# VIS4ROB-lab/ccm_slam

Hardware: AMD Instinct MI355X
Metric: global-BA LM iterations/s (4-agent merged map) (higher is better)
Workload: dtype f64; 1 GPU; gba_c4: global BA (MapFusionGBA numerics), 2000 KFs / 150000 landmarks / 954782 observations, Huber sqrt(5.99), landmark-sharded x1

## Files before the change

ccm_slam_amd/csrc/ba.hip:

```cpp
#include "common.h"
#include "test_internal.h"
#include "ba_types.h"
#include "lane_xor.h"
#include "ba_math.h"
#include <algorithm>
#include <chrono>
#include <cmath>
#include <cstring>
#include <limits>
#include <numeric>

int ccm_allreduce_f64(ccm_ctx* ctx, double* d_buf, size_t n);
int ccm_allreduce_max_f64(ccm_ctx* ctx, double* d_buf, size_t n);

namespace {


inline double now_ms() {
  return std::chrono::duration<double, std::milli>(std::chrono::steady_clock::now().time_since_epoch()).count();
}

__device__ __forceinline__ double wave_sum(double v) { return lanex::wave_sum(v); }

__device__ __forceinline__ double block_sum(double v, double* lds ) {
// ... 218 lines not shown
      for (int k = 0; k < 12; k++) Jj[k] = 0.0;
    }
    if (d.E4) {
      v2d* E = reinterpret_cast<v2d*>(d.E4 + 4 * (size_t)s);
      v2d ea, eb; ea[0] = Xc[0]; ea[1] = Xc[1]; eb[0] = off ? 0.0 : iz; eb[1] = wom;
      E[0] = ea; E[1] = eb;
    }
    int k = 0;
#pragma unroll
    for (int a = 0; a < 6; a++)
#pragma unroll
      for (int b = a; b < 6; b++) acc[k++] += (Jj[a] * Jj[b] + Jj[6 + a] * Jj[6 + b]) * wom;
#pragma unroll
    for (int a = 0; a < 6; a++) acc[21 + a] += Jj[a] * o0 + Jj[6 + a] * o1;
  }
  const double tot = wave_sum27(acc, lane);
  if ((lane & 1) == 0) {
    const int k = lane >> 1;
    if (k < 21) { int a, b; tri_ab(k, a, b); double* H = d.Hpp + 36 * (size_t)i; H[a * 6 + b] = tot; H[b * 6 + a] = tot; }
    else if (k < 27) d.bp[6 * (size_t)i + k - 21] = tot;
  }
}

__global__ __launch_bounds__(kTPB) void ba_maxdiag(BaDev d, const double* hpp_full, double* partial, int n_partial, int final) {
  __shared__ double lds[kTPB];
  double m = 0;
  if (!final) {
    const int stride = gridDim.x * kTPB;
    for (int i = blockIdx.x * kTPB + threadIdx.x; i < d.Cp * 6; i += stride) m = fmax(m, fabs(hpp_full[36 * (size_t)(i / 6) + (i % 6) * 7]));
    for (int i = blockIdx.x * kTPB + threadIdx.x; i < d.Lloc * 3; i += stride) {
      const int l = i / 3, k = i % 3;
      m = fmax(m, fabs(d.Hll[6 * (size_t)l + (k == 0 ? 0 : (k == 1 ? 3 : 5))]));
    }
  } else {
    for (int i = threadIdx.x; i < n_partial; i += kTPB) m = fmax(m, partial[i]);
  }
  lds[threadIdx.x] = m;
  __syncthreads();
  for (int s = kTPB / 2; s > 0; s >>= 1) {
    if (threadIdx.x < s) lds[threadIdx.x] = fmax(lds[threadIdx.x], lds[threadIdx.x + s]);
    __syncthreads();
  }
  if (threadIdx.x == 0) { if (final) d.scal[4] = lds[0]; else partial[blockIdx.x] = lds[0]; }
}

__global__ __launch_bounds__(kTPB) void ba_dinv(BaDev d, double lambda) {
  const int l = blockIdx.x * blockDim.x + threadIdx.x;
  if (l >= d.Lloc) return;
  double a[6], r[6];
#pragma unroll
  for (int i = 0; i < 6; i++) a[i] = d.Hll[6 * (size_t)l + i];
  a[0] += lambda; a[3] += lambda; a[5] += lambda;
  ba_sym3_inv(a, r);
#pragma unroll
  for (int i = 0; i < 6; i++) d.Dinv[6 * (size_t)l + i] = r[i];
  const double b0 = d.bl[3 * (size_t)l], b1 = d.bl[3 * (size_t)l + 1], b2 = d.bl[3 * (size_t)l + 2];
  d.dl[3 * (size_t)l] = r[0] * b0 + r[1] * b1 + r[2] * b2;
  d.dl[3 * (size_t)l + 1] = r[1] * b0 + r[3] * b1 + r[4] * b2;
  d.dl[3 * (size_t)l + 2] = r[2] * b0 + r[4] * b1 + r[5] * b2;
}

__global__ __launch_bounds__(kTPB) void ba_schur_diag(BaDev d) {
  const int lane = threadIdx.x & (kWave - 1);
  const int i = blockIdx.x * (kTPB / kWave) + threadIdx.x / kWave;
  if (i >= d.Cp) return;
  double acc[32];
// ... 788 lines not shown
  Ac[idx] = sum;
}

constexpr long kPersMaxSpins = 8000;
constexpr int kPersCooldownTrials = 8;

struct PersArgs {
  double lambda, rel_tol;
  int max_it, n_clu;
  unsigned* bar;
  int test_abort;
  const int* coff; const int* cij; const uint32_t* cblk;
  unsigned long long* slots;
  unsigned long long* utag;
  unsigned long long* tag;
  int prefetch;
  unsigned long long epoch_base;
  const int* uoff;
  const int* ucol;
  const int* loc;
  long long* dbg;
  const double* Ainv; const double* Pm; int na, Nc;
  double* wsave; int w_load;
};

__device__ __forceinline__ double pers_uniform(double v) {
  const long long b = __double_as_longlong(v);
  const int lo = __builtin_amdgcn_readfirstlane((int)(b & 0xffffffffll)), hi = __builtin_amdgcn_readfirstlane((int)(b >> 32));
  return __longlong_as_double(((long long)hi << 32) | (unsigned int)lo);
}

typedef unsigned int pers_u32x4 __attribute__((ext_vector_type(4)));
constexpr int kAuxSc1 = 16;
__device__ __forceinline__ void tag_store(__amdgpu_buffer_rsrc_t rs, unsigned byte_off, double v, unsigned long long key) {
  const unsigned long long b = (unsigned long long)__double_as_longlong(v), c = b ^ key;
  pers_u32x4 q;
  q.x = (unsigned)b; q.y = (unsigned)(b >> 32); q.z = (unsigned)c; q.w = (unsigned)(c >> 32);
  __builtin_amdgcn_raw_buffer_store_b128(q, rs, (int)byte_off, 0, kAuxSc1);
}
__device__ __forceinline__ pers_u32x4 tag_load(__amdgpu_buffer_rsrc_t rs, unsigned byte_off) { return __builtin_amdgcn_raw_buffer_load_b128(rs, (int)byte_off, 0, kAuxSc1); }
__device__ __forceinline__ bool tag_valid(pers_u32x4 q, unsigned long long key) {
  return (q.x ^ q.z) == (unsigned)key && (q.y ^ q.w) == (unsigned)(key >> 32);
}
__device__ __forceinline__ double tag_value(pers_u32x4 q) { return __longlong_as_double((long long)(((unsigned long long)q.y << 32) | q.x)); }

template <class Mid>
// ... 673 lines not shown
  {
    double sc = 0;
    if (t < Cp) {
      const int c = d.slot_cam[t];
      double u[6];
#pragma unroll
      for (int q = 0; q < 6; q++) u[q] = xv[6 * t + q];
      const BaPose Tc = ba_load_pose(d.cam[cur] + 7 * (size_t)c);
      const BaPose Tn = ba_oplus(u, Tc);
      ba_store_pose(d.cam[cur ^ 1] + 7 * (size_t)c, Tn);
#pragma unroll
      for (int q = 0; q < 6; q++) sc += u[q] * ((add_lambda_term ? lambda * u[q] : 0.0) + d.bp[6 * (size_t)t + q]);
    }
    if (t < kWave) {
      const double s = wave_sum(sc);
      if (t == 0) d.part_cam[0] = ((s + 0.0) + 0.0) + 0.0;
    }
  }
  CR_TICK(3)
  if (dbg && t == 0) dbg[7] += 1;
#undef CR_TICK
#undef CR_TIJ
  if (t == 0) { d.pcg_flag[0] = 1; d.pcg_flag[1] = 1; d.pcg_flag[2] = ibuf[1]; d.pcg_flag[3] = 0; }
}

__global__ __launch_bounds__(kPersTPB) void ba_pcg_persist(BaDev d, PersArgs a) {
  extern __shared__ __attribute__((aligned(16))) double sm[];
  constexpr int N = kCluN;
  double* A = sm;
  double* Li = sm + N * N;
  double* rc = Li + N * N;
  double* xs = rc + N;
  double* ps = xs + N / 2;
  double* ss = ps + N / 2;
  double* zs = ss + N;
  double* zpart = zs + N;
  double* wl = zpart + 4 * N;
  double* pso = zpart + 8 * N;
  double* red = pso + kPersNcCap;
  int* ibuf = reinterpret_cast<int*>(red + 2 * kPersWaves + 4);
  if (a.test_abort && blockIdx.x == gridDim.x - 1) return;
  const int t = threadIdx.x, lane = t & (kWave - 1);
  const int wv = __builtin_amdgcn_readfirstlane(t / kWave);
  const int nwg = gridDim.x;
  const int per_xcd = nwg >> 3;
  const int u = (blockIdx.x & 7) * per_xcd + (blockIdx.x >> 3);
// ... 51 lines not shown
  } else {
    pers_factor_cluster(A, Li, ibuf, a.cij, a.cblk, has ? a.coff[c] : 0, has ? a.coff[c + 1] : 0, d.S, s0, s1, lambda, has, tacc, timing);
    double wreg[5];
    int nw = 0;
    for (int e = t; e < N * (N / 2); e += kPersTPB, nw++) wreg[nw] = A[(e / (N / 2)) * N + ob + e % (N / 2)];
    __syncthreads();
    nw = 0;
    double* dst = a.wsave ? a.wsave + (size_t)u * (N * (N / 2)) : nullptr;
    for (int e = t; e < N * (N / 2); e += kPersTPB, nw++) { A[e] = wreg[nw]; if (dst) dst[e] = wreg[nw]; }
  }
  const int Nc = a.Nc, nca = 6 * (a.na + 1);
  float* ainv_l = reinterpret_cast<float*>(A + N * (N / 2));
  double* rco = Li + (32 + 2 * kPersIdxCap + kPersColCap) / 2 + 6 * kPersColCap + 256;
  double* pown = rco + Nc;
  double* ypart = pown + 8 * 36;
  constexpr int kParkA = 8 * N - (4 * N + N / 2);
  double* park_a = zpart + 4 * N + N / 2;
  double* park_b = ypart + 12;
  auto park = [&](int x) { return x < kParkA ? park_a + x : park_b + (x - kParkA); };
  static_assert((32 + 2 * kPersIdxCap + kPersColCap) % 2 == 0 &&
                (32 + 2 * kPersIdxCap + kPersColCap) / 2 + 6 * kPersColCap + 256 + kPersNcCap + 8 * 36 + 12 + (N + kPersNcCap - kParkA) <= kCluN * kCluN,
                "coarse vectors and the parked values do not fit behind the staged structure");
  if (coarse) {
    {
      const double* src = a.Ainv + (size_t)(6 * agg) * Nc;
      double tmpa[9];
#pragma unroll
      for (int q = 0; q < 9; q++) { const int e = t + q * kPersTPB; tmpa[q] = (has && e < 12 * Nc) ? src[e] : 0.0; }
#pragma unroll
      for (int q = 0; q < 9; q++) { const int e = t + q * kPersTPB; if (e < 12 * Nc) ainv_l[e] = (float)tmpa[q]; }
    }
    for (int e = t; e < Nc; e += kPersTPB) { rco[e] = 0.0; pso[e] = 0.0; }
    for (int e = t; e < 8 * 36; e += kPersTPB) pown[e] = (e / 36 < nown) ? a.Pm[36 * (size_t)o0 + e] : 0.0;
  }
  __syncthreads();
  auto fetch_pre = [&](unsigned long long e, bool want_w) {
    const unsigned long long key = key_of(e);
    int tf = tq;
    asm volatile("" : "+v"(tf));
    const int p = tf - kWave, j = p - N;
    const bool is_w = want_w && p >= 0 && p < m && !(p >= ob && p < ob + mo);
    const bool is_c = coarse && j >= 0 && j < nca;
    const int n = j / 6;
    bool ok = true;
    double sgm = 0;
    for (int h = 0; h < 2 && 2 * h < aggu; h++) {
      unsigned off[2] = {c_off(e, 2 * h, j), c_off(e, 4 + 2 * h, j)}, want = 0;
// ... 215 lines not shown
    __syncthreads();
    PERS_TICK(0)
    const double ru_t = apply_W(key_of(epoch + 1));
    PERS_TICK(1)
    long long tw0 = 0;
    if (a.dbg && t == 0) tw0 = wall_clock64();
    alive = halo_load(key_of(epoch + 1));
    if (a.dbg && t == 0) a.dbg[33 + 2 * u] += wall_clock64() - tw0;
    PERS_TICK(2)
    if (!alive) { fail = 1; break; }
    double wu_t = 0;
    spmv_w(epoch + 1, &wu_t);
    if (coarse) { __syncthreads(); coarse_restrict(pown, wl, epoch + 1); }
    PERS_TICK(3)
    gam_prev = gam; alpha_prev = alpha;
    if (a.dbg && t == 0) tw0 = wall_clock64();
    alive = exchange(epoch + 1, ru_t, wu_t, false, &gam, &del);
    ++epoch;
    if (a.dbg && t == 0) a.dbg[32 + 2 * u] += wall_clock64() - tw0;
    PERS_TICK(4)
    if (!alive) { fail = 1; break; }
  }
#undef PERS_TICK
  if (timing) { for (int q = 0; q < 12; q++) a.dbg[q] += tacc[q]; a.dbg[12] += k; a.dbg[13] += 1; }
  if (t < mo) d.x[6 * (size_t)o0 + t] = xs[t];
  if (blockIdx.x == 0 && t == 0) {
    d.pcg_flag[0] = 1; d.pcg_flag[1] = k; d.pcg_flag[2] = fail;
    d.pcg_flag[3] = ibuf[2] | (int)__hip_atomic_load(a.bar + 1, __ATOMIC_RELAXED, __HIP_MEMORY_SCOPE_AGENT);
  }
}

__global__ __launch_bounds__(kPersTPB) void ba_pcg_init_tiles(BaDev d, double lambda, double rel_tol, const int* coff, const int* cij, const uint32_t* cblk) {
  extern __shared__ __attribute__((aligned(16))) double sm[];
  constexpr int N = kCluN;
  double* A = sm;
  double* Li = sm + N * N;
  double* rc = Li + N * N;
  double* red = rc + N;
  int* ibuf = reinterpret_cast<int*>(red + kPersWaves);
  const int t = threadIdx.x, c = blockIdx.x;
  const int s0 = c * kClu, s1 = min(d.Cp, s0 + kClu);
  const int m = 6 * (s1 - s0);
  if (t < 4) ibuf[t] = 0;
  __syncthreads();
  pers_factor_cluster(A, Li, ibuf, cij, cblk, coff[c], coff[c + 1], d.S, s0, s1, lambda, true, nullptr, false);
  float* W = d.Wc + (size_t)c * N * N;
  for (int e = t; e < N * N; e += kPersTPB) W[e] = (float)A[e];
// ... 15 lines not shown
    for (int w = 0; w < kPersWaves; w++) tot += red[w];
    d.prz[0][c] = tot;
    d.prz[1][c] = 0;
    if (ibuf[1]) d.pcg_flag[2] = 1;
    if (c == 0) { d.pcg_scal[1] = rel_tol * rel_tol; d.pcg_scal[2] = lambda; }
  }
  if (d.mk_on) mk_restrict(d, c, s0, m, rc, Li);
}

constexpr size_t kPersLdsBytes = (size_t)(2 * kCluN * kCluN + 4 * kCluN + 8 * kCluN + kPersNcCap + 2 * kPersWaves + 4) * sizeof(double) + 16 + 14 * sizeof(long long);
static_assert(kPersLdsBytes <= 160 * 1024, "persistent PCG: LDS of one workgroup exceeds the 160 KB of a CU");
static inline size_t pers_lds_bytes() { return kPersLdsBytes; }

static PersArgs pers_args(ccm_ba* ba, double lambda, double rel_tol, int max_it) {
  PersArgs pa{};
  pa.lambda = lambda; pa.rel_tol = rel_tol; pa.max_it = max_it; pa.n_clu = ccm_div_up(ba->d.Cp, kClu);
  pa.bar = ba->d_pers_bar; pa.slots = (unsigned long long*)ba->d_pers_part;
  pa.utag = (unsigned long long*)ba->d_pers_u; pa.tag = ba->d_pers_tag; pa.prefetch = ba->pers_prefetch ? 1 : 0;
  pa.epoch_base = (++ba->pers_launch) << 20;
  pa.uoff = ba->d_pers_uoff; pa.ucol = ba->d_pers_ucol; pa.loc = ba->d_pers_loc;
  pa.coff = ba->d_pers_coff; pa.cij = ba->d_pers_cij; pa.cblk = ba->d_pers_cblk;
  return pa;
}
static void pers_args_coarse(const ccm_ba* ba, PersArgs* pa) { pa->Ainv = ba->d_cAinv; pa->Pm = ba->d_cP; pa->na = ba->coarse_na; pa->Nc = ba->coarse_Nc; }


template <int TPB>
__device__ __forceinline__ double block_dot_small(double v, double* red ) {
  v = wave_sum(v);
  if (TPB == kWave) return v;
  __syncthreads();
  if ((threadIdx.x & (kWave - 1)) == 0) red[threadIdx.x / kWave] = v;
  __syncthreads();
  double s = 0;
#pragma unroll
  for (int i = 0; i < TPB / kWave; i++) s += red[i];
  return s;
}

template <int kSmallTPB>
__global__ __launch_bounds__(kSmallTPB) void ba_pcg_small(BaDev d, double lambda, double rel_tol, int max_it, int stage_S, int n_entries) {
  extern __shared__ __attribute__((aligned(16))) double sm[];
  const int n = 6 * d.Cp;
  double* xs = sm; double* rs = xs + n; double* zs = rs + n; double* ps = zs + n; double* qs = ps + n;
  double* Mi = qs + n;
  double* red = Mi + 36 * d.Cp;
  double* Sl = red + 18;
// ... 205 lines not shown
    }
    Xs[t][0] = X[0]; Xs[t][1] = X[1]; Xs[t][2] = X[2];
  }
  __syncthreads();
  if (t < ne) {
    const int e = e0 + t, c = d.ed_cam[e], ll = d.ed_pt[e] - l0;
    const double X[3] = {Xs[ll][0], Xs[ll][1], Xs[ll][2]};
    const BaPose T = ba_load_pose(d.cam[trial] + 7 * (size_t)c);
    const double K4[4] = {d.K[4 * c], d.K[4 * c + 1], d.K[4 * c + 2], d.K[4 * c + 3]};
    double r0, r1;
    const double zc = ba_residual(T, K4, X, d.obs[2 * (size_t)e], d.obs[2 * (size_t)e + 1], r0, r1);
    const double c2 = d.info[e] != 0.0 ? (r0 * r0 + r1 * r1) * d.info[e] : 0.0;
    double rho0, w;
    ba_huber(c2, d.huber, rho0, w);
    chi = rho0;
    if (d.info[e] != 0.0) d.edge_chi2[e] = c2;
    d.edge_depth[e] = zc > 0.0;
  }
  const double s0 = block_sum(chi, lds);
  const double s1 = block_sum(sc, lds);
  if (threadIdx.x == 0) { d.part_pt[2 * blockIdx.x] = s0; d.part_pt[2 * blockIdx.x + 1] = s1; }
}

__global__ __launch_bounds__(kTPB) void ba_reduce_scalars(BaDev d, int stop_local, int abort_local, int pers_trial, double* h_out, unsigned long long ticket) {
  __shared__ double lds[kTPB / kWave];
  double chi = 0, sc = 0;
  for (int i = threadIdx.x; i < d.n_part; i += kTPB) { chi += d.part_pt[2 * i]; sc += d.part_pt[2 * i + 1]; }
  for (int i = threadIdx.x; i < d.n_wg_cam; i += kTPB) sc += d.part_cam[i];
  const double a = block_sum(chi, lds);
  const double b = block_sum(sc, lds);
  if (threadIdx.x == 0) {
    d.scal[0] = a; d.scal[1] = b;
    d.scal[2] = stop_local ? 1.0 : 0.0;
    const double s3 = abort_local ? 4096.0 : (pers_trial && d.pcg_flag[3]) ? 1.0 : 0.0;
    d.scal[3] = s3;
    if (h_out) {
      h_out[0] = a; h_out[1] = b; h_out[2] = stop_local ? 1.0 : 0.0; h_out[3] = s3;
      h_out[4] = d.scal[4]; h_out[5] = d.scal[5]; h_out[6] = d.scal[6]; h_out[7] = d.scal[7];
      __hip_atomic_store(reinterpret_cast<unsigned long long*>(h_out) + 8, ticket, __ATOMIC_RELEASE, __HIP_MEMORY_SCOPE_SYSTEM);
    }
  }
}

__global__ void ba_scatter_points(double* full, const double* own, int lb , int Lloc) {
  const int l = blockIdx.x * blockDim.x + threadIdx.x;
  if (l >= Lloc) return;
  const int g = lb + l;
  full[3 * (size_t)g] = own[3 * (size_t)l]; full[3 * (size_t)g + 1] = own[3 * (size_t)l + 1]; full[3 * (size_t)g + 2] = own[3 * (size_t)l + 2];
}

}


namespace {

template <typename T>
int dev_upload(ccm_ba* ba, const std::vector<T>& v, T** out) {
  ccm_ctx* ctx = ba->ctx;
// ... 164 lines not shown
      if (spin == 0xffff) t_start = now_ms();
      else if (now_ms() - t_start > 2000.0) break;
    }
#if defined(__x86_64__)
    __builtin_ia32_pause();
#endif
  }
  if (!got) return read_scalars(ba, out, flags);
  __atomic_thread_fence(__ATOMIC_ACQUIRE);
  memcpy(out, ba->h_rb, 6 * sizeof(double));
  if (flags) memcpy(flags, ba->h_rb + 6, 4 * sizeof(int));
  CCM_HIP_CHECK(ba->ctx, hipGetLastError());
  return CCM_OK;
}

int eval_chi2(ccm_ba* ba, double* chi) {
  ccm_ctx* ctx = ba->ctx;
  BaDev& d = ba->d;
  {
    ccm_prof_scope ps(ctx, CCM_K_BA_CHI2);
    if (d.chunk_off) hipLaunchKernelGGL(ba_backsub_chi2_e, dim3(d.n_chunk), dim3(kTPB), 0, ctx->stream, d, ba->cur, 0.0, 1);
    else hipLaunchKernelGGL(ba_backsub_chi2, dim3(d.n_wg_pt), dim3(kTPB), 0, ctx->stream, d, ba->cur, 0.0, 1);
  }
  hipMemsetAsync(d.part_cam, 0, sizeof(double) * d.n_wg_cam, ctx->stream);
  const bool poll = ba->nranks == 1 && poll_enabled();
  const unsigned long long ticket = ++ba->rb_ticket;
  hipLaunchKernelGGL(ba_reduce_scalars, dim3(1), dim3(kTPB), 0, ctx->stream, d, ba->stop_local(), 0, 0, poll ? ba->h_rb : (double*)nullptr, ticket);
  RC(ba_allreduce_sum(ba, d.scal, 4));
  double s[6];
  if (poll) { RC(read_scalars_polled(ba, s, nullptr, ticket)); } else { RC(read_scalars(ba, s)); }
  *chi = s[0];
  ba->stop_any = s[2] > 0.0;
  return CCM_OK;
}

int build_system(ccm_ba* ba, double lambda_next = -1.0) {
  ccm_ctx* ctx = ba->ctx;
  BaDev& d = ba->d;
  ba->dinv_done_lambda = -1.0;
  if (d.Lloc) {
    ccm_prof_scope ps(ctx, CCM_K_BA_LINEARIZE);
    if (d.chunk_off) {
      hipLaunchKernelGGL(ba_linearize_pts_e, dim3(d.n_chunk), dim3(kTPB), 0, ctx->stream, d, ba->cur, lambda_next);
      if (lambda_next >= 0.0) ba->dinv_done_lambda = lambda_next;
    } else hipLaunchKernelGGL(ba_linearize_pts, dim3(d.n_wg_pt), dim3(kTPB), 0, ctx->stream, d, ba->cur);
  }
  if (d.Cp) {
    ccm_prof_scope ps(ctx, CCM_K_BA_CAM);
    hipLaunchKernelGGL(ba_linearize_cams, dim3(d.n_wg_wave4), dim3(kTPB), 0, ctx->stream, d, ba->cur);
  }
  CCM_HIP_CHECK(ctx, hipGetLastError());
  return CCM_OK;
}

int max_diag(ccm_ba* ba, double* out) {
  ccm_ctx* ctx = ba->ctx;
  BaDev& d = ba->d;
  const double* hpp = d.Hpp;
  if (ba->nranks > 1 && d.Cp) {
    CCM_HIP_CHECK(ctx, hipMemcpyAsync(ba->d_hpp_full, d.Hpp, 36 * (size_t)d.Cp * sizeof(double), hipMemcpyDeviceToDevice, ctx->stream));
    RC(ba_allreduce_sum(ba, ba->d_hpp_full, 36 * (size_t)d.Cp));
    hpp = ba->d_hpp_full;
  }
  const int nb = std::max(1, std::min(d.n_wg_pt, 512));
  hipLaunchKernelGGL(ba_maxdiag, dim3(nb), dim3(kTPB), 0, ctx->stream, d, hpp, d.part_pt, nb, 0);
  hipLaunchKernelGGL(ba_maxdiag, dim3(1), dim3(kTPB), 0, ctx->stream, d, hpp, d.part_pt, nb, 1);
  RC(ba_allreduce_max(ba, d.scal + 4, 1));
  double s[6];
  RC(read_scalars(ba, s));
  *out = s[4];
  return CCM_OK;
}

__global__ void ba_f64_to_f32(const double* __restrict__ in, float* __restrict__ out, size_t n) {
  const size_t i = (size_t)blockIdx.x * blockDim.x + threadIdx.x;
  if (i < n) out[i] = (float)in[i];
}

int coarse_build(ccm_ba* ba, double lambda) {
  ccm_ctx* ctx = ba->ctx;
  BaDev& d = ba->d;
  ccm_prof_scope ps(ctx, CCM_K_BA_COARSE);
  const int Nc = ba->coarse_Nc, na = ba->coarse_na, nn = na + 1;
  hipLaunchKernelGGL(ba_coarse_P, dim3(ccm_div_up(d.Cp, kTPB)), dim3(kTPB), 0, ctx->stream, d, ba->cur, ba->d_cP);
  hipLaunchKernelGGL(ba_coarse_assemble, dim3(ba->coarse_ncb), dim3(kCoarseTPB), 0, ctx->stream, d, (const double*)ba->d_cP,
                     (const int*)ba->d_cb_off, (const int*)ba->d_cb_ent, ba->coarse_ncb, (const int*)ba->d_blk_i, (const int*)ba->d_blk_j, lambda, ba->d_cstage);
  hipLaunchKernelGGL(ba_coarse_sum, dim3(ccm_div_up((int64_t)Nc * Nc, kTPB)), dim3(kTPB), 0, ctx->stream, (const double*)ba->d_cstage, (const unsigned*)ba->d_cb_key,
                     ba->coarse_ncb, na, nn, ba->d_cA, Nc);
  CCM_HIP_CHECK(ctx, hipGetLastError());
  RC(ccm_dense_chol_inverse_dev(ctx, ba->d_cA, Nc, ba->d_cLinv, ba->d_cX, ba->d_cAinv, ba->d_cinfo));
  if (ba->d_cAinv32) {
    const size_t n = (size_t)Nc * Nc;
// ... 57 lines not shown
        hipLaunchKernelGGL(ba_solve_dense2, dim3(1), dim3(kPersTPB), dense2_lds_bytes(), ctx->stream, d, lambda, (const int*)ba->d_pers_coff, (const int*)ba->d_pers_cij,
                           (const uint32_t*)ba->d_pers_cblk, ba->d_dense_T,
                           ccm_dbg("dense2") ? (long long*)(ba->d_dense_T + kCluN * kCluN) : (long long*)nullptr, cur, ba->rank == 0 ? 1 : 0);
      }
      small_path = true;
      cams_updated = true;
    } else if (d.Cp <= kSmallMaxCp) {
      size_t lds = (size_t)(5 * 6 * d.Cp + 36 * d.Cp + 18) * sizeof(double);
      const size_t lds_S = 36 * (size_t)(d.Cp + d.nOff) * sizeof(double) + ((size_t)d.Cp + 1 + 2 * (size_t)ba->n_row_entries) * sizeof(int) + 16;
      const int stage_S = (lds + lds_S <= 150 * 1024) ? 1 : 0;
      if (stage_S) lds += lds_S;
      CCM_LDS_ATTR(ctx, CCM_LDS_BA_SMALL, ba_pcg_small<1024>, 150 * 1024);
      {
        ccm_prof_scope ps(ctx, CCM_K_BA_PCG_SPMV);
        hipLaunchKernelGGL(ba_pcg_small<1024>, dim3(1), dim3(1024), lds, ctx->stream, d, lambda, tol, max_it, stage_S, (int)ba->n_row_entries);
      }
      small_path = true;
    } else {
    bool persist_ok = false;
    if (ba->pers_grid) {
      PersArgs pa = pers_args(ba, lambda, tol, max_it);
      pa.test_abort = getenv("CCM_BA_TEST_ABORT") ? 1 : 0;
      pa.dbg = ccm_dbg("pers") ? (long long*)(ba->d_pers_bar + 4) : nullptr;
      const int w_mode = 1;
      const double w_win = 8.5;
      pa.wsave = ba->d_pers_wsave;
      {
        const bool same_lin = ba->w_lin_id == ba->lin_id;
        const bool in_win = ba->w_lambda_built > 0 && lambda <= w_win * ba->w_lambda_built && lambda >= ba->w_lambda_built / w_win;
        const bool reuse = ba->d_pers_wsave && w_mode > 0 && ba->w_valid && in_win && !pa.test_abort && (same_lin || (w_mode >= 2 && !ba->w_stale_bad));
        pa.w_load = reuse ? 1 : 0;
        ba->w_loaded = reuse;
        if (!reuse) { ba->w_valid = false; ba->w_pending = ba->d_pers_wsave != nullptr; ba->w_lambda_built = lambda; ba->w_lin_id = ba->lin_id; ba->w_stale_bad = false; }
      }
      const double coarse_lmax = 1.0;
      const bool damped = ba->coarse_force == 0 && coarse_lmax > 0 && ba->lambda_first > 0 && lambda >= coarse_lmax * ba->lambda_first;
      const bool use_coarse = ba->coarse_na && !damped && (ba->coarse_force > 0 || (ba->coarse_force == 0 && ba->coarse_active));
      ba->coarse_used = use_coarse;
      ba->coarse_skipped_damped = damped;
      if (use_coarse) {
        if (ccm_dbg("coarse")) {
          hipStreamSynchronize(ctx->stream); const double tc0 = now_ms();
          RC(coarse_prepare(ba, lambda));
          const double tc1 = now_ms(); hipStreamSynchronize(ctx->stream);
          fprintf(stderr, "[ccm_ba] coarse_build: enqueue %.3f ms, complete %.3f ms\n", tc1 - tc0, now_ms() - tc0);
        } else
        RC(coarse_prepare(ba, lambda));
        pers_args_coarse(ba, &pa);
      }
      static const bool trial_dbg = ccm_dbg("trial");
      double tdbg0 = 0;
      if (trial_dbg) { hipStreamSynchronize(ctx->stream); tdbg0 = now_ms(); }
      {
        ccm_coresident_scope lease(ctx);
        ccm_prof_scope ps(ctx, CCM_K_BA_PCG_PERSIST);
        hipLaunchKernelGGL(ba_pcg_persist, dim3(ba->pers_grid), dim3(kPersTPB), pers_lds_bytes(), ctx->stream, d, pa);
        const hipError_t le = hipGetLastError();
        if (le == hipSuccess) persist_ok = true;
        else { (void)hipGetLastError(); ba->pers_grid = 0; ba->pers_grid_built = 0; ba->w_valid = false; pers_launch_failed = true; }
      }
      if (persist_ok) small_path = pers_trial = true;
      if (trial_dbg) {
        hipStreamSynchronize(ctx->stream);
        int fl[4] = {0, 0, 0, 0};
        hipMemcpy(fl, d.pcg_flag, sizeof(fl), hipMemcpyDeviceToHost);
        fprintf(stderr, "[ccm_ba] trial: lin %d lambda %.4g persist %.1f us, %d CG iterations, coarse %s, W %s\n", ba->lin_id, lambda, (now_ms() - tdbg0) * 1e3, fl[1],
                !use_coarse ? "off" : ba->coarse_fresh ? "built" : "reused", pa.w_load ? "loaded" : "factored");
      }
    }
    if (!persist_ok) {
      d.mk_on = 0;
      const double coarse_lmax_mk = 1.0;
      const bool damped_mk = ba->coarse_force == 0 && coarse_lmax_mk > 0 && ba->lambda_first > 0 && lambda >= coarse_lmax_mk * ba->lambda_first;
      ba->coarse_skipped_damped = damped_mk;
      if (d.mk_cpart && ba->coarse_na && !damped_mk && (ba->coarse_force > 0 || (ba->coarse_force == 0 && ba->coarse_active))) {
        RC(coarse_prepare(ba, lambda));
        d.mk_on = 1;
      }
      ba->coarse_used = d.mk_on != 0;
      CCM_HIP_CHECK(ctx, hipMemsetAsync(d.pcg_flag, 0, 4 * sizeof(int), ctx->stream));
      if (d.S32) {
        const size_t n4 = 9 * (size_t)(d.Cp + d.nOff);
        hipLaunchKernelGGL(ba_s_to_f32, dim3((unsigned)ccm_div_up((int64_t)n4, kTPB)), dim3(kTPB), 0, ctx->stream, (const double*)d.S, d.S32, n4);
      }
// ... 41 lines not shown
        if (flags[0]) {
          const int N = flags[1];
          if (f32 && !flags[2] && N > 0 && N % kMkReplaceEvery != 0 && verified_at != N) {
            verified_at = N;
            CCM_HIP_CHECK(ctx, hipMemsetAsync(d.pcg_flag, 0, 2 * sizeof(int), ctx->stream));
            replace_residual(N - 1);
            k = N;
            after_verify = true;
            flags[0] = 0;
            continue;
          }
          break;
        }
      }
      *pcg_iters = flags[0] ? flags[1] : k;
      ba->mk_prev_iters = *pcg_iters;
    }
    }
    if (flags[2]) *ok = false;
  }
  if (d.Cp && !cams_updated) {
    ccm_prof_scope ps(ctx, CCM_K_BA_UPDATE);
    hipLaunchKernelGGL(ba_update_cams, dim3(d.n_wg_cam), dim3(kTPB), 0, ctx->stream, d, cur, lambda, ba->rank == 0 ? 1 : 0, ba->d_pers_bar );
  } else if (!d.Cp) hipMemsetAsync(d.part_cam, 0, sizeof(double) * d.n_wg_cam, ctx->stream);
  {
    ccm_prof_scope ps(ctx, CCM_K_BA_BACKSUB);
    if (d.chunk_off) hipLaunchKernelGGL(ba_backsub_chi2_e, dim3(d.n_chunk), dim3(kTPB), 0, ctx->stream, d, cur, lambda, 0);
    else hipLaunchKernelGGL(ba_backsub_chi2, dim3(d.n_wg_pt), dim3(kTPB), 0, ctx->stream, d, cur, lambda, 0);
  }
  const bool poll = ba->nranks == 1 && poll_enabled();
  const unsigned long long ticket = ++ba->rb_ticket;
  {
    ccm_prof_scope ps(ctx, CCM_K_BA_REDUCE);
    hipLaunchKernelGGL(ba_reduce_scalars, dim3(1), dim3(kTPB), 0, ctx->stream, d, ba->stop_local(), (pers_launch_failed && ba->nranks > 1) ? 1 : 0,
                       pers_trial ? 1 : 0, poll ? ba->h_rb : (double*)nullptr, ticket);
  }
  RC(ba_allreduce_sum(ba, d.scal, 4));
  double s[6];
  if (poll) { RC(read_scalars_polled(ba, s, small_flags, ticket)); } else { RC(read_scalars(ba, s, small_flags)); }
  CCM_HIP_CHECK(ctx, hipGetLastError());
  ba->stop_any = s[2] > 0.0;
  if (s[3] > 0.0) {
    if (pers_trial) { ccm_coresident_note_abort(ctx); ba->pers_aborts++; }
    ba->pers_grid = 0; ba->pers_cooldown = kPersCooldownTrials;
    if (ba->nranks > 1 && s[3] >= 4096.0) ba->pers_grid_built = 0;
    ba->w_valid = false; ba->w_pending = false;
    return lm_trial(ba, lambda, opt, temp_chi, scale, ok, pcg_iters);
  }
  if (small_path) { *pcg_iters = small_flags[1]; if (small_flags[2]) *ok = false; }
  if (pers_trial) {
    if (!ba->w_loaded) ba->w_fresh_iters = *pcg_iters;
    else if (ba->w_lin_id != ba->lin_id && *pcg_iters > ba->w_fresh_iters + ba->w_fresh_iters / 8 + 3) ba->w_stale_bad = true;
    if (ba->w_pending) { ba->w_valid = !small_flags[2]; ba->w_pending = false; }
    if (small_flags[2]) ba->w_valid = false;
  }
  if (ba->coarse_na && (small_path || d.mk_cpart)) {
    if (ba->coarse_used) {
      if (ba->coarse_fresh) ba->coarse_fresh_iters = *pcg_iters;
// ... 102 lines not shown
    long long h[11];
    hipMemcpy(h, ba->d_dense_T + kCluN * kCluN, sizeof(h), hipMemcpyDeviceToHost);
    const double nl = (double)std::max<long long>(h[8], 1);
    fprintf(stderr, "[ccm_ba] exact two-cluster solve: %lld launches; us/launch: assemble1 %.1f factor1 %.1f t1+A12 %.1f T %.1f P+c %.1f assemble2 %.1f factor2 %.1f x %.1f | both factorisations: cholesky %.1f inverse-factor %.1f\n", h[8],
            h[0] * 0.01 / nl, h[1] * 0.01 / nl, h[2] * 0.01 / nl, h[3] * 0.01 / nl, h[4] * 0.01 / nl, h[5] * 0.01 / nl, h[6] * 0.01 / nl, h[7] * 0.01 / nl, h[9] * 0.01 / nl, h[10] * 0.01 / nl);
  }
  if (!ba->pers_grid || !ccm_dbg("pers")) return;
  long long h[16];
  hipMemcpy(h, ba->d_pers_bar + 4, sizeof(h), hipMemcpyDeviceToHost);
  {
    std::vector<long long> w(2 * (size_t)ba->pers_grid);
    hipMemcpy(w.data(), (long long*)(ba->d_pers_bar + 4) + 32, w.size() * sizeof(long long), hipMemcpyDeviceToHost);
    const double itn = (double)std::max<long long>(h[12], 1);
    for (int x = 0; x < 2; x++) {
      std::vector<double> v;
      for (int g = 0; g < ba->pers_grid; g++) if (w[2 * g + x] > 0) v.push_back(w[2 * g + x] * 0.01 / itn);
      std::sort(v.begin(), v.end());
      if (!v.empty()) fprintf(stderr, "[ccm_ba] persistent PCG, %s per unit and iteration (us): min %.2f  p10 %.2f  median %.2f  p90 %.2f  max %.2f  (%zu units)\n",
                              x == 0 ? "time inside the exchange" : "halo wait", v.front(), v[v.size() / 10], v[v.size() / 2], v[v.size() * 9 / 10], v.back(), v.size());
    }
  }
  const double it = (double)std::max<long long>(h[12], 1), nl = (double)std::max<long long>(h[13], 1);
  fprintf(stderr, "[ccm_ba] persistent PCG, workgroup 0: %lld iterations in %lld launches; us/iteration: update %.2f W %.2f halo %.2f "
          "spmv+dot %.2f exchange %.2f | us/launch: assemble %.1f cholesky %.1f inverse %.1f W %.1f start %.1f\n",
          h[12], h[13], h[0] * 0.01 / it, h[1] * 0.01 / it, h[2] * 0.01 / it, h[3] * 0.01 / it, h[4] * 0.01 / it,
          h[7] * 0.01 / nl, h[8] * 0.01 / nl, h[9] * 0.01 / nl, h[10] * 0.01 / nl, h[11] * 0.01 / nl);
}

extern "C" int ccm_ba_run(ccm_ba* ba, const ccm_ba_options* opt_in, const volatile unsigned char* stop_flag, ccm_ba_stats* stats) {
  if (!ba) return CCM_E_ARG;
  ccm_ctx* ctx = ba->ctx;
  if (ba->nranks > 1 && ((!ctx->comm && !ctx->loop_group) || ctx->comm_nranks != ba->nranks || ctx->comm_rank != ba->rank))
    return ccm_set_error(ctx, CCM_E_STATE, "ccm_ba_run: sharded problem needs a matching communicator (ccm_comm_init)");
  CCM_HIP_CHECK(ctx, hipSetDevice(ctx->device));
  ccm_ba_options opt{};
  if (opt_in) opt = *opt_in;
  ba->coarse_active = false;
  ba->mk_prev_iters = 0;
  ba->coarse_valid = false; ba->coarse_stale_bad = false; ba->coarse_fresh_iters = 0;
  ba->w_valid = false; ba->w_stale_bad = false; ba->w_fresh_iters = 0; ba->w_lambda_built = 0; ba->lin_id = 0; ba->w_lin_id = -1;
  ba->stop_flag = stop_flag; ba->stop_any = false;
  ba->hist_chi2.clear(); ba->hist_lambda.clear(); ba->hist_trials.clear();
  if (ba->nranks > 1 && !ba->pers_agreed) {
    const double mine = ba->pers_grid ? 0.0 : 1.0;
    CCM_HIP_CHECK(ctx, hipMemcpyAsync(ba->d.scal + 5, &mine, sizeof(double), hipMemcpyHostToDevice, ctx->stream));
    CCM_HIP_CHECK(ctx, hipStreamSynchronize(ctx->stream));
    RC(ba_allreduce_max(ba, ba->d.scal + 5, 1));
    double any = 0;
    CCM_HIP_CHECK(ctx, hipMemcpyAsync(&any, ba->d.scal + 5, sizeof(double), hipMemcpyDeviceToHost, ctx->stream));
// ... 201 lines not shown
```

ccm_slam_amd/csrc/ba_build.hip:

```cpp
#include "common.h"
#include "ba_types.h"
#include "ba_math.h"
#include "ba_sort.h"
#include <algorithm>
#include <chrono>
#include <cstring>
#include <rocprim/rocprim.hpp>

int ccm_ba_build_pairs(ccm_ctx* ctx, const int* d_pt_off, const int* d_cslot, int Lp, int Cp, int lb, int le, int eb,
                       uint32_t** d_U_out, int* nOff_out, int** d_inst_off, int** d_inst_a, int** d_inst_c, int64_t* n_inst,
                       std::vector<std::pair<void*, size_t>>& keep);
int ccm_ba_pers_grid_fits(ccm_ctx* ctx, int grid);
int ccm_ba_state_from_raw(ccm_ba* ba);

namespace {

constexpr int kB = 256;

inline double now_ms() { return std::chrono::duration<double, std::milli>(std::chrono::steady_clock::now().time_since_epoch()).count(); }

struct BuildSizes {
  int Cp, Lp, Eact, bad, max_cam_edges, n_fix_edges, worst_units, n_units, pers_bad, n_ucol, n_cij, ncb, pad[4];
};

// ... 743 lines not shown
    memset(ba->h_rb, 0, 128);
    ba->red_count = 36 * (size_t)(Cp + nOff) + 6 * (size_t)Cp;
    BB_RC(keep_get(ba, ba->red_count, &ba->d_red, true));
    d.S = ba->d_red; d.bs = ba->d_red + 36 * (size_t)(Cp + nOff);
    BB_RC(keep_get(ba, 3 * (size_t)std::max(Lp, 1), &ba->d_pt_full, true));
    BB_RC(keep_get(ba, 36 * (size_t)std::max(Cp, 1), &ba->d_hpp_full, true));
    auto coarse_buffers = [&]() -> int {
      BB_RC(keep_get(ba, 36 * (size_t)Cp, &ba->d_cP, true));
      BB_RC(keep_get(ba, (size_t)Nc * Nc, &ba->d_cA, true)); BB_RC(keep_get(ba, (size_t)Nc * Nc, &ba->d_cX, true));
      BB_RC(keep_get(ba, (size_t)Nc * Nc, &ba->d_cAinv, true)); BB_RC(keep_get(ba, (size_t)Nc * 64, &ba->d_cLinv, true));
      BB_RC(keep_get(ba, 4, &ba->d_cinfo, true));
      ba->coarse_na = na; ba->coarse_Nc = Nc; ba->coarse_ncb = hs.ncb;
      if (const char* cf = getenv("CCM_BA_COARSE")) ba->coarse_force = !strcmp(cf, "always") ? 1 : !strcmp(cf, "never") ? -1 : 0;
      return CCM_OK;
    };
    ba->pers_grid = 0;
    d.mk_cpart = nullptr; d.mk_cry[0] = d.mk_cry[1] = nullptr; d.mk_P = nullptr; d.mk_Ainv = nullptr; d.mk_Ainv32 = nullptr; d.mk_on = 0; d.mk_Nc = 0; d.mk_na = 0;
    if (pers_try && !hs.pers_bad) {
      BB_RC(keep_get(ba, 4 + 2 * 16 + 4 * 512, &ba->d_pers_bar, true));
      BB_RC(keep_get(ba, 8 * (size_t)pers_grid_want, &ba->d_pers_part, true));
      BB_RC(keep_get(ba, 12 * (size_t)Cp, &ba->d_pers_u, true));
      BB_RC(keep_get(ba, 2 * (2 * 6 * (size_t)Cp + 2 * 8 * (size_t)kPersNcCap), &ba->d_pers_tag, true));
      { const char* pf = getenv("CCM_BA_PERS_PREFETCH"); ba->pers_prefetch = !(pf && !strcmp(pf, "0")); }
      ba->pers_grid = pers_grid_want; ba->pers_grid_built = pers_grid_want;
      BB_RC(keep_get(ba, (size_t)pers_grid_want * (kCluN * (kCluN / 2)), &ba->d_pers_wsave, false));
      if (coarse_pers) BB_RC(coarse_buffers());
    } else if (pers_try) { ba->d_pers_uoff = nullptr; ba->d_pers_ucol = nullptr; ba->d_pers_loc = nullptr; }
    if (Cp > kSmallMaxCp && Cp <= kDense2MaxCp && ba->d_pers_coff)
      BB_RC(keep_get(ba, (size_t)kCluN * kCluN + 16, &ba->d_dense_T, true));
    if (cholreg_win) {
      const size_t np = 16 * (size_t)ccm_div_up(6 * Cp, 16);
      BB_RC(keep_get(ba, 16, &ba->d_cholreg_dbg, true));
      BB_RC(keep_get(ba, np * np, &ba->d_cholreg_L, false));
      BB_RC(keep_get(ba, (size_t)8 * 24 * 64 * 4, &ba->d_cholreg_tab, false));
    }
    if (!ba->pers_grid && coarse_mk) {
      BB_RC(coarse_buffers());
      double *p1 = nullptr, *p2 = nullptr, *p3 = nullptr;
      BB_RC(keep_get(ba, 24 * (size_t)(na + 1), &p1, true)); BB_RC(keep_get(ba, (size_t)n_cl, &p2, true)); BB_RC(keep_get(ba, (size_t)n_cl, &p3, true));
      d.mk_cpart = p1; d.mk_cry[0] = p2; d.mk_cry[1] = p3;
      d.mk_P = ba->d_cP; d.mk_Ainv = ba->d_cAinv; d.mk_Nc = Nc; d.mk_na = na;
      BB_RC(keep_get(ba, (size_t)Nc * Nc, &ba->d_cAinv32, false)); d.mk_Ainv32 = ba->d_cAinv32;
    }
    d.S32 = nullptr; d.qx = nullptr;
    if (!ba->pers_grid && pers_wanted && pers_grid_want > 4 * kWave) {
      float* p32 = nullptr;
      BB_RC(keep_get(ba, 36 * (size_t)(Cp + nOff), &p32, false));
      d.S32 = p32;
      double* pqx = nullptr;
// ... 17 lines not shown
```

ccm_slam_amd/csrc/ba_types.h:

```cpp
#pragma once
#include "common.h"

constexpr int kWave = 64;
constexpr int kTPB = 256;
constexpr uint32_t kTransposeBit = 0x80000000u;
constexpr int kRowMaxEdges = 1000;
constexpr int kRow2TPB = 1024;
constexpr int kRow2Group = 16;
constexpr int kRow2Chunk = 64;
constexpr int kClu = 16;
constexpr int kCluN = 6 * kClu;
constexpr int kSpmvTPB = 1024;
constexpr int kRowsPerWG = kSpmvTPB / (2 * kWave);
constexpr int kCoarseNcCap = 768;
constexpr int kAggFine = 16, kAggMid = 24, kAggWide = 32;
constexpr int kPersTPB = 1024;
constexpr int kPersWaves = kPersTPB / kWave;
constexpr int kPersIdxCap = 3072;
constexpr int kPersColCap = 640;
constexpr int kPersNcCap = 768;
constexpr int kSmallMaxCp = 16;
constexpr int kDense2MaxCp = 2 * kClu;
constexpr int kCholRegMaxCp = 50;

struct BaDev {
  int n_cam, Cp, Lloc, Eloc, nOff;
  double huber;
  double* cam[2];
  const double* K;
  const int* slot_cam;
  double* pt[2];
  const int* pt_off;
  const int* ed_cam;
  const int* ed_cslot;
  const int* ed_pt;
  const double* obs;
  const double* info;
  const int* cam_off;
  const int* cam_edge;
  const int* cam_pt;
  double* cam_oi;
  double* W;
  double* Hll;
  double* bl;
  double* Dinv;
// ... 15 lines not shown
  const int* blk_unit0;
  int row_units_max;
  int unit_chunk;
  double* E4;
  double* E4L;
  int w_free;
  double* camRK;
  const int* inst_cp;
  const int* blk_j;
  long long* row_dbg;
  const int* row_off;
  const int* row_col;
  const uint32_t* row_blk;
  double *x, *r, *z, *q, *p[2];
  float* Wc;
  double *ppq, *prz[2];
  double* pcg_scal;
  int* pcg_flag;
  int n_wg_spmv, n_wg_upd, n_wg_wave4;
  double* edge_chi2;
  uint8_t* edge_depth;
  double* part_pt;
  double* part_cam;
  double* scal;
  int n_wg_pt, n_wg_cam;
  const int* chunk_off;
  int n_chunk;
  int n_part;
  double* mk_cpart;
  double* mk_cry[2];
  const double* mk_P;
  const double* mk_Ainv;
  const float* mk_Ainv32;
  int mk_on, mk_Nc, mk_na;
  int agg;
};

struct ccm_ba {
  ccm_ctx* ctx = nullptr;
  int rank = 0, nranks = 1;
  int n_cam = 0, n_pt = 0, n_edge = 0;
  int Cp = 0, Lp = 0, Lloc = 0, Eloc = 0, nOff = 0;
  int64_t n_inst = 0, n_act_edges = 0, n_row_entries = 0;
  int lp_begin = 0, lp_end = 0;
  std::vector<int> slot_cam;
  std::vector<int> loc_edge_orig;
// ... 2 lines not shown
  std::vector<std::pair<void*, size_t>> allocs;
  std::vector<std::pair<void*, size_t>> zero_list;
  BaDev d{};
  int cur = 0;
  double* d_red = nullptr; size_t red_count = 0;
  unsigned* d_pers_bar = nullptr; double* d_pers_part = nullptr; int pers_grid = 0;
  double* d_dense_T = nullptr;
  double* d_cholreg_dbg = nullptr;
  int* d_cholreg_tab = nullptr;
  bool cholreg_table_built = false;
  double* d_cholreg_L = nullptr;
  int *d_pers_uoff = nullptr, *d_pers_ucol = nullptr, *d_pers_loc = nullptr, *d_pers_coff = nullptr, *d_pers_cij = nullptr;
  uint32_t* d_pers_cblk = nullptr;
  unsigned long long pers_launch = 0;
  int pers_grid_built = 0, pers_cooldown = 0, pers_aborts = 0;
  bool w_pending = false;
  bool pers_agreed = false;
  int coarse_na = 0, coarse_Nc = 0, coarse_ncb = 0;
  bool coarse_active = false, coarse_used = false;
  double* d_pers_wsave = nullptr;
  double* d_pers_u = nullptr;
  unsigned long long* d_pers_tag = nullptr;
  bool pers_prefetch = true;
  float* d_cAinv32 = nullptr;
  bool w_valid = false, w_loaded = false, w_stale_bad = false; double w_lambda_built = 0; int w_fresh_iters = 0, lin_id = 0, w_lin_id = -1;
  bool coarse_valid = false, coarse_fresh = false, coarse_stale_bad = false, coarse_reuse = true;
  double coarse_lambda_built = 0; int coarse_fresh_iters = 0;
  int mk_prev_iters = 0;
  double dinv_done_lambda = -1.0;
  double lambda_first = 0; bool coarse_skipped_damped = false;
  double* h_rb = nullptr;
  unsigned long long rb_ticket = 0;
  int coarse_force = 0;
  double *d_cP = nullptr, *d_cA = nullptr, *d_cX = nullptr, *d_cAinv = nullptr, *d_cLinv = nullptr;
  unsigned* d_cb_key = nullptr;
  double* d_cstage = nullptr;
  int *d_cb_off = nullptr, *d_cb_ent = nullptr, *d_cb_ab = nullptr, *d_blk_i = nullptr, *d_blk_j = nullptr, *d_cinfo = nullptr;
  double* d_pt_full = nullptr;
  double* d_hpp_full = nullptr;
  double *d_saved_cam = nullptr, *d_saved_pt = nullptr;
  double* d_info_orig = nullptr;
  double ms_setup = 0;
  const volatile unsigned char* stop_flag = nullptr;
  bool stop_any = false;
  bool stop_requested() const { return nranks > 1 ? stop_any : (stop_flag && *stop_flag); }
  int stop_local() const { return (stop_flag && *stop_flag) ? 1 : 0; }
// ... 4 lines not shown
```

Baseline: 1012 LM iter/s.

## Fuse camera pose update into persistent PCG kernel and poll max-diagonal readback

Moves the camera pose update (oplus plus scale term) into the tail of the persistent PCG kernel so the separate ba_update_cams launch is skipped. The per-camera scale terms are written to a new buffer and summed inside the reduce kernel. The reduce kernel also zeroes the persistent flags, which removes the part_cam memsets. The reduce kernel now loads part_pt as batched double2 values, the max-diagonal readback uses host polling instead of a blocking read, and the coarse Ainv load can take a float32 copy. The cost is extra branches and a dependence on n_wg_cam staying within 16 blocks.

```diff
diff --git a/ccm_slam_amd/csrc/ba.hip b/ccm_slam_amd/csrc/ba.hip
--- a/ccm_slam_amd/csrc/ba.hip
+++ b/ccm_slam_amd/csrc/ba.hip
@@ -264,7 +264,7 @@
   }
 }
 
-__global__ __launch_bounds__(kTPB) void ba_maxdiag(BaDev d, const double* hpp_full, double* partial, int n_partial, int final) {
+__global__ __launch_bounds__(kTPB) void ba_maxdiag(BaDev d, const double* hpp_full, double* partial, int n_partial, int final, double* h_out, unsigned long long ticket) {
   __shared__ double lds[kTPB];
   double m = 0;
   if (!final) {
@@ -283,7 +283,13 @@
     if (threadIdx.x < s) lds[threadIdx.x] = fmax(lds[threadIdx.x], lds[threadIdx.x + s]);
     __syncthreads();
   }
-  if (threadIdx.x == 0) { if (final) d.scal[4] = lds[0]; else partial[blockIdx.x] = lds[0]; }
+  if (threadIdx.x == 0) {
+    if (!final) partial[blockIdx.x] = lds[0];
+    else {
+      d.scal[4] = lds[0];
+      if (h_out) { h_out[4] = lds[0]; __hip_atomic_store(reinterpret_cast<unsigned long long*>(h_out) + 8, ticket, __ATOMIC_RELEASE, __HIP_MEMORY_SCOPE_SYSTEM); }
+    }
+  }
 }
 
 __global__ __launch_bounds__(kTPB) void ba_dinv(BaDev d, double lambda) {
@@ -1118,6 +1124,8 @@
   long long* dbg;
   const double* Ainv; const double* Pm; int na, Nc;
   double* wsave; int w_load;
+  int cam_upd, cur, add_lambda_term;
+  const float* Ainv32;
 };
 
 __device__ __forceinline__ double pers_uniform(double v) {
@@ -1837,6 +1845,24 @@
 #undef CR_TICK
 #undef CR_TIJ
   if (t == 0) { d.pcg_flag[0] = 1; d.pcg_flag[1] = 1; d.pcg_flag[2] = ibuf[1]; d.pcg_flag[3] = 0; }
+}
+
+__device__ __noinline__ void pers_update_cams(const double* xs, int o0, int nown, const int* slot_cam, const double* cam_in, double* cam_out, const double* bp,
+                                              double* cam_sc, double lambda, int add_lambda_term) {
+  const int t = threadIdx.x;
+  if (t >= nown) return;
+  const int i = o0 + t;
+  const int c = slot_cam[i];
+  double u[6];
+#pragma unroll
+  for (int q = 0; q < 6; q++) u[q] = xs[6 * t + q];
+  const BaPose T = ba_load_pose(cam_in + 7 * (size_t)c);
+  const BaPose Tn = ba_oplus(u, T);
+  ba_store_pose(cam_out + 7 * (size_t)c, Tn);
+  double sc = 0;
+#pragma unroll
+  for (int q = 0; q < 6; q++) sc += u[q] * ((add_lambda_term ? lambda * u[q] : 0.0) + bp[6 * (size_t)i + q]);
+  cam_sc[i] = sc;
 }
 
 __global__ __launch_bounds__(kPersTPB) void ba_pcg_persist(BaDev d, PersArgs a) {
@@ -1934,7 +1960,14 @@
                 (32 + 2 * kPersIdxCap + kPersColCap) / 2 + 6 * kPersColCap + 256 + kPersNcCap + 8 * 36 + 12 + (N + kPersNcCap - kParkA) <= kCluN * kCluN,
                 "coarse vectors and the parked values do not fit behind the staged structure");
   if (coarse) {
-    {
+    if (a.Ainv32) {
+      const float* src = a.Ainv32 + (size_t)(6 * agg) * Nc;
+      float tmpa[9];
+#pragma unroll
+      for (int q = 0; q < 9; q++) { const int e = t + q * kPersTPB; tmpa[q] = (has && e < 12 * Nc) ? src[e] : 0.0f; }
+#pragma unroll
+      for (int q = 0; q < 9; q++) { const int e = t + q * kPersTPB; if (e < 12 * Nc) ainv_l[e] = tmpa[q]; }
+    } else {
       const double* src = a.Ainv + (size_t)(6 * agg) * Nc;
       double tmpa[9];
 #pragma unroll
@@ -2196,7 +2229,9 @@
     if (!alive) { fail = 1; break; }
   }
 #undef PERS_TICK
-  if (timing) { for (int q = 0; q < 12; q++) a.dbg[q] += tacc[q]; a.dbg[12] += k; a.dbg[13] += 1; }
+  if (timing) tacc[12] = wall_clock64();
+  if (a.cam_upd && wv == 0) pers_update_cams(xs, o0, nown, d.slot_cam, a.cur ? d.cam[1] : d.cam[0], a.cur ? d.cam[0] : d.cam[1], d.bp, d.cam_sc, lambda, a.add_lambda_term);
+  if (timing) { tacc[5] += wall_clock64() - tacc[12]; for (int q = 0; q < 12; q++) a.dbg[q] += tacc[q]; a.dbg[12] += k; a.dbg[13] += 1; }
   if (t < mo) d.x[6 * (size_t)o0 + t] = xs[t];
   if (blockIdx.x == 0 && t == 0) {
     d.pcg_flag[0] = 1; d.pcg_flag[1] = k; d.pcg_flag[2] = fail;
@@ -2258,7 +2293,7 @@
   pa.coff = ba->d_pers_coff; pa.cij = ba->d_pers_cij; pa.cblk = ba->d_pers_cblk;
   return pa;
 }
-static void pers_args_coarse(const ccm_ba* ba, PersArgs* pa) { pa->Ainv = ba->d_cAinv; pa->Pm = ba->d_cP; pa->na = ba->coarse_na; pa->Nc = ba->coarse_Nc; }
+static void pers_args_coarse(const ccm_ba* ba, PersArgs* pa) { pa->Ainv = ba->d_cAinv; pa->Ainv32 = ba->d_cAinv32; pa->Pm = ba->d_cP; pa->na = ba->coarse_na; pa->Nc = ba->coarse_Nc; }
 
 
 template <int TPB>
@@ -2510,11 +2545,42 @@
   if (threadIdx.x == 0) { d.part_pt[2 * blockIdx.x] = s0; d.part_pt[2 * blockIdx.x + 1] = s1; }
 }
 
-__global__ __launch_bounds__(kTPB) void ba_reduce_scalars(BaDev d, int stop_local, int abort_local, int pers_trial, double* h_out, unsigned long long ticket) {
+constexpr int kRedCamNone = 0, kRedCamPart = 1, kRedCamTerms = 2;
+constexpr int kRedBatch = 8;
+__global__ __launch_bounds__(kTPB) void ba_reduce_scalars(BaDev d, int stop_local, int abort_local, int pers_trial, int cam_mode, unsigned* pers_flags, double* h_out,
+                                                          unsigned long long ticket) {
   __shared__ double lds[kTPB / kWave];
+  __shared__ double cam_ws[kRedCamBlocks][kTPB / kWave];
   double chi = 0, sc = 0;
-  for (int i = threadIdx.x; i < d.n_part; i += kTPB) { chi += d.part_pt[2 * i]; sc += d.part_pt[2 * i + 1]; }
-  for (int i = threadIdx.x; i < d.n_wg_cam; i += kTPB) sc += d.part_cam[i];
+  double cs[kRedCamBlocks];
+  if (cam_mode == kRedCamTerms) {
+#pragma unroll
+    for (int q = 0; q < kRedCamBlocks; q++) { const int i = q * kTPB + (int)threadIdx.x; cs[q] = (q < d.n_wg_cam && i < d.Cp) ? d.cam_sc[i] : 0.0; }
+  }
+  const double2* pp = reinterpret_cast<const double2*>(d.part_pt);
+  for (int i0 = threadIdx.x; i0 < d.n_part; i0 += kRedBatch * kTPB) {
+    double2 v[kRedBatch];
+#pragma unroll
+    for (int q = 0; q < kRedBatch; q++) { const int i = i0 + q * kTPB; v[q] = (i < d.n_part) ? pp[i] : double2{0.0, 0.0}; }
+#pragma unroll
+    for (int q = 0; q < kRedBatch; q++) if (i0 + q * kTPB < d.n_part) { chi += v[q].x; sc += v[q].y; }
+  }
+  if (cam_mode == kRedCamTerms) {
+#pragma unroll
+    for (int q = 0; q < kRedCamBlocks; q++) if (q < d.n_wg_cam) cs[q] = wave_sum(cs[q]);
+    if ((threadIdx.x & (kWave - 1)) == 0) {
+#pragma unroll
+      for (int q = 0; q < kRedCamBlocks; q++) if (q < d.n_wg_cam) cam_ws[q][threadIdx.x / kWave] = cs[q];
+    }
+    __syncthreads();
+    if ((int)threadIdx.x < d.n_wg_cam && threadIdx.x < kRedCamBlocks) {
+      double s = 0;
+      for (int i = 0; i < kTPB / kWave; i++) s += cam_ws[threadIdx.x][i];
+      sc += s;
+    }
+  } else if (cam_mode == kRedCamPart) {
+    for (int i = threadIdx.x; i < d.n_wg_cam; i += kTPB) sc += d.part_cam[i];
+  }
   const double a = block_sum(chi, lds);
   const double b = block_sum(sc, lds);
   if (threadIdx.x == 0) {
@@ -2522,6 +2588,7 @@
     d.scal[2] = stop_local ? 1.0 : 0.0;
     const double s3 = abort_local ? 4096.0 : (pers_trial && d.pcg_flag[3]) ? 1.0 : 0.0;
     d.scal[3] = s3;
+    if (pers_flags) { pers_flags[0] = 0u; pers_flags[1] = 0u; pers_flags[2] = 0u; pers_flags[3] = 0u; }
     if (h_out) {
       h_out[0] = a; h_out[1] = b; h_out[2] = stop_local ? 1.0 : 0.0; h_out[3] = s3;
       h_out[4] = d.scal[4]; h_out[5] = d.scal[5]; h_out[6] = d.scal[6]; h_out[7] = d.scal[7];
@@ -2732,10 +2799,10 @@
     if (d.chunk_off) hipLaunchKernelGGL(ba_backsub_chi2_e, dim3(d.n_chunk), dim3(kTPB), 0, ctx->stream, d, ba->cur, 0.0, 1);
     else hipLaunchKernelGGL(ba_backsub_chi2, dim3(d.n_wg_pt), dim3(kTPB), 0, ctx->stream, d, ba->cur, 0.0, 1);
   }
-  hipMemsetAsync(d.part_cam, 0, sizeof(double) * d.n_wg_cam, ctx->stream);
   const bool poll = ba->nranks == 1 && poll_enabled();
   const unsigned long long ticket = ++ba->rb_ticket;
-  hipLaunchKernelGGL(ba_reduce_scalars, dim3(1), dim3(kTPB), 0, ctx->stream, d, ba->stop_local(), 0, 0, poll ? ba->h_rb : (double*)nullptr, ticket);
+  hipLaunchKernelGGL(ba_reduce_scalars, dim3(1), dim3(kTPB), 0, ctx->stream, d, ba->stop_local(), 0, 0, kRedCamNone ,
+                     (unsigned*)nullptr, poll ? ba->h_rb : (double*)nullptr, ticket);
   RC(ba_allreduce_sum(ba, d.scal, 4));
   double s[6];
   if (poll) { RC(read_scalars_polled(ba, s, nullptr, ticket)); } else { RC(read_scalars(ba, s)); }
@@ -2773,11 +2840,14 @@
     hpp = ba->d_hpp_full;
   }
   const int nb = std::max(1, std::min(d.n_wg_pt, 512));
-  hipLaunchKernelGGL(ba_maxdiag, dim3(nb), dim3(kTPB), 0, ctx->stream, d, hpp, d.part_pt, nb, 0);
-  hipLaunchKernelGGL(ba_maxdiag, dim3(1), dim3(kTPB), 0, ctx->stream, d, hpp, d.part_pt, nb, 1);
+  const bool poll = ba->nranks == 1 && poll_enabled();
+  const unsigned long long ticket = poll ? ++ba->rb_ticket : 0ull;
+  hipLaunchKernelGGL(ba_maxdiag, dim3(nb), dim3(kTPB), 0, ctx->stream, d, hpp, d.part_pt, nb, 0, (double*)nullptr, 0ull);
+  hipLaunchKernelGGL(ba_maxdiag, dim3(1), dim3(kTPB), 0, ctx->stream, d, hpp, d.part_pt, nb, 1, poll ? ba->h_rb : (double*)nullptr, ticket);
+  CCM_HIP_CHECK(ctx, hipGetLastError());
   RC(ba_allreduce_max(ba, d.scal + 4, 1));
   double s[6];
-  RC(read_scalars(ba, s));
+  if (poll) { RC(read_scalars_polled(ba, s, nullptr, ticket)); } else { RC(read_scalars(ba, s)); }
   *out = s[4];
   return CCM_OK;
 }
@@ -2881,6 +2951,7 @@
       PersArgs pa = pers_args(ba, lambda, tol, max_it);
       pa.test_abort = getenv("CCM_BA_TEST_ABORT") ? 1 : 0;
       pa.dbg = ccm_dbg("pers") ? (long long*)(ba->d_pers_bar + 4) : nullptr;
+      pa.cam_upd = ba->pers_camupd ? 1 : 0; pa.cur = cur; pa.add_lambda_term = ba->rank == 0 ? 1 : 0;
       const int w_mode = 1;
       const double w_win = 8.5;
       pa.wsave = ba->d_pers_wsave;
@@ -2918,7 +2989,7 @@
         if (le == hipSuccess) persist_ok = true;
         else { (void)hipGetLastError(); ba->pers_grid = 0; ba->pers_grid_built = 0; ba->w_valid = false; pers_launch_failed = true; }
       }
-      if (persist_ok) small_path = pers_trial = true;
+      if (persist_ok) { small_path = pers_trial = true; cams_updated = pa.cam_upd != 0; }
       if (trial_dbg) {
         hipStreamSynchronize(ctx->stream);
         int fl[4] = {0, 0, 0, 0};
@@ -3006,7 +3077,7 @@
   if (d.Cp && !cams_updated) {
     ccm_prof_scope ps(ctx, CCM_K_BA_UPDATE);
     hipLaunchKernelGGL(ba_update_cams, dim3(d.n_wg_cam), dim3(kTPB), 0, ctx->stream, d, cur, lambda, ba->rank == 0 ? 1 : 0, ba->d_pers_bar );
-  } else if (!d.Cp) hipMemsetAsync(d.part_cam, 0, sizeof(double) * d.n_wg_cam, ctx->stream);
+  }
   {
     ccm_prof_scope ps(ctx, CCM_K_BA_BACKSUB);
     if (d.chunk_off) hipLaunchKernelGGL(ba_backsub_chi2_e, dim3(d.n_chunk), dim3(kTPB), 0, ctx->stream, d, cur, lambda, 0);
@@ -3017,7 +3088,8 @@
   {
     ccm_prof_scope ps(ctx, CCM_K_BA_REDUCE);
     hipLaunchKernelGGL(ba_reduce_scalars, dim3(1), dim3(kTPB), 0, ctx->stream, d, ba->stop_local(), (pers_launch_failed && ba->nranks > 1) ? 1 : 0,
-                       pers_trial ? 1 : 0, poll ? ba->h_rb : (double*)nullptr, ticket);
+                       pers_trial ? 1 : 0, !d.Cp ? kRedCamNone : (pers_trial && cams_updated) ? kRedCamTerms : kRedCamPart,
+                       ba->d_pers_bar , poll ? ba->h_rb : (double*)nullptr, ticket);
   }
   RC(ba_allreduce_sum(ba, d.scal, 4));
   double s[6];
@@ -3166,9 +3238,9 @@
   }
   const double it = (double)std::max<long long>(h[12], 1), nl = (double)std::max<long long>(h[13], 1);
   fprintf(stderr, "[ccm_ba] persistent PCG, workgroup 0: %lld iterations in %lld launches; us/iteration: update %.2f W %.2f halo %.2f "
-          "spmv+dot %.2f exchange %.2f | us/launch: assemble %.1f cholesky %.1f inverse %.1f W %.1f start %.1f\n",
+          "spmv+dot %.2f exchange %.2f | us/launch: assemble %.1f cholesky %.1f inverse %.1f W %.1f start %.1f camera update %.2f\n",
           h[12], h[13], h[0] * 0.01 / it, h[1] * 0.01 / it, h[2] * 0.01 / it, h[3] * 0.01 / it, h[4] * 0.01 / it,
-          h[7] * 0.01 / nl, h[8] * 0.01 / nl, h[9] * 0.01 / nl, h[10] * 0.01 / nl, h[11] * 0.01 / nl);
+          h[7] * 0.01 / nl, h[8] * 0.01 / nl, h[9] * 0.01 / nl, h[10] * 0.01 / nl, h[11] * 0.01 / nl, h[5] * 0.01 / nl);
 }
 
 extern "C" int ccm_ba_run(ccm_ba* ba, const ccm_ba_options* opt_in, const volatile unsigned char* stop_flag, ccm_ba_stats* stats) {
diff --git a/ccm_slam_amd/csrc/ba_build.hip b/ccm_slam_amd/csrc/ba_build.hip
--- a/ccm_slam_amd/csrc/ba_build.hip
+++ b/ccm_slam_amd/csrc/ba_build.hip
@@ -789,9 +789,15 @@
       BB_RC(keep_get(ba, 12 * (size_t)Cp, &ba->d_pers_u, true));
       BB_RC(keep_get(ba, 2 * (2 * 6 * (size_t)Cp + 2 * 8 * (size_t)kPersNcCap), &ba->d_pers_tag, true));
       { const char* pf = getenv("CCM_BA_PERS_PREFETCH"); ba->pers_prefetch = !(pf && !strcmp(pf, "0")); }
+      {
+        const char* cu = getenv("CCM_BA_PERS_CAMUPD");
+        ba->pers_camupd = !(cu && !strcmp(cu, "0")) && d.n_wg_cam <= kRedCamBlocks;
+        double* p_sc = nullptr;
+        BB_RC(keep_get(ba, (size_t)Cp, &p_sc, true)); d.cam_sc = p_sc;
+      }
       ba->pers_grid = pers_grid_want; ba->pers_grid_built = pers_grid_want;
       BB_RC(keep_get(ba, (size_t)pers_grid_want * (kCluN * (kCluN / 2)), &ba->d_pers_wsave, false));
-      if (coarse_pers) BB_RC(coarse_buffers());
+      if (coarse_pers) { BB_RC(coarse_buffers()); BB_RC(keep_get(ba, (size_t)Nc * Nc, &ba->d_cAinv32, false)); }
     } else if (pers_try) { ba->d_pers_uoff = nullptr; ba->d_pers_ucol = nullptr; ba->d_pers_loc = nullptr; }
     if (Cp > kSmallMaxCp && Cp <= kDense2MaxCp && ba->d_pers_coff)
       BB_RC(keep_get(ba, (size_t)kCluN * kCluN + 16, &ba->d_dense_T, true));
diff --git a/ccm_slam_amd/csrc/ba_types.h b/ccm_slam_amd/csrc/ba_types.h
--- a/ccm_slam_amd/csrc/ba_types.h
+++ b/ccm_slam_amd/csrc/ba_types.h
@@ -21,6 +21,7 @@
 constexpr int kPersNcCap = 768;
 constexpr int kSmallMaxCp = 16;
 constexpr int kDense2MaxCp = 2 * kClu;
+constexpr int kRedCamBlocks = 16;
 constexpr int kCholRegMaxCp = 50;
 
 struct BaDev {
@@ -82,6 +83,7 @@
   uint8_t* edge_depth;
   double* part_pt;
   double* part_cam;
+  double* cam_sc;
   double* scal;
   int n_wg_pt, n_wg_cam;
   const int* chunk_off;
@@ -130,6 +132,7 @@
   double* d_pers_u = nullptr;
   unsigned long long* d_pers_tag = nullptr;
   bool pers_prefetch = true;
+  bool pers_camupd = true;
   float* d_cAinv32 = nullptr;
   bool w_valid = false, w_loaded = false, w_stale_bad = false; double w_lambda_built = 0; int w_fresh_iters = 0, lin_id = 0, w_lin_id = -1;
   bool coarse_valid = false, coarse_fresh = false, coarse_stale_bad = false, coarse_reuse = true;
```

Result: no change. 1025 LM iter/s, median of 6 (+1.2%).
